# peter-seres/python-ray-tracer

Measured on AMD Instinct MI355X. Metric: Mrays/sec + frame time (ms) at 1920x1080, 8 spheres, depth=3, higher is better.
Workload: dtype f64

## Files before the change

python-ray-tracer_amd/csrc/rt_device.h:

```cpp
#pragma once
#include <hip/hip_runtime.h>
#include <stdint.h>
#include "rt_kparams.h"
#include "rt_math.h"
#include "rt_facing.h"
#include "rt_layout.h"

#pragma clang fp contract(off)

#ifndef RT_FAST_DIVSQRT
#define RT_FAST_DIVSQRT 1
#endif
#ifndef RT_FAST_NORMALIZE
#define RT_FAST_NORMALIZE 1
#endif
#ifndef RT_FACING_SKIP
#define RT_FACING_SKIP 1
#endif

namespace rt {

constexpr int TABLE_THREADS = 256;

__device__ __forceinline__ int div_by(int n, int d, unsigned M, unsigned sh)
// ... 662 lines not shown
    constexpr bool F32 = MODE >= 1;
    if (MODE >= 2 && lds.NC > 0 && (canchor < 0 || p.lanes_primary)) {
        if (canchor >= 0) lanes_closest<true>(lds, p, canchor, o, R, a, bestn, bidx);
        else lanes_closest<false>(lds, p, -1, o, R, a, bestn, bidx);
    } else
    for (int k0 = 0; k0 < S; k0 += 64) {
      const int n = (S - k0 < 64) ? S - k0 : 64;
      unsigned long long mask = cull_mask(lds, S, canchor, k0, n, o, R, p.extent2, -1);
      mask &= (n == 64) ? ~0ull : ((1ull << n) - 1ull);
      RT_MARK(1);
      while (mask) {
        const int k = k0 + __builtin_ctzll(mask);
        mask &= mask - 1ull;
        sphere_closest<F32>(lds, p, k, o, R, a, bestn, bidx);
      }
      RT_MARK(2);
    }
    double best = 999.0;
    int idx = -1, type = HIT_NONE;
    if (bidx >= 0) {
        const double t = div_inrange(bestn, a);
        if (best > t && t > 0.0) { best = t; idx = bidx; type = HIT_SPHERE; }
    }
    const double *pl = lds.recs() + (F32 ? 0 : opaque(p.S) * SPH_STRIDE);
    for (int k = 0; k < P; ++k) {
        const double *g = pl + k * PL_STRIDE;
        double den, num;
        plane_den_num(g, plane_code(p, k), o, d, den, num, lds.trim);
        if (!(__builtin_fabs(den) < 0.001)) {
            const double t = div_inrange(num, den);
            if (best > t && t > 0.0) { best = t; idx = k; type = HIT_PLANE; }
        }
    }
    t_out = best; idx_out = idx; type_out = type;
    RT_MARK(3);
}

__device__ __forceinline__ bool any_hit_masks(const Lds &lds, const KParams &p, const V3 &o, const V3 &d, int anchor, int self)
{
    const int P = opaque(p.P);
    const int S = p.S;
    const V3 R = renormalize_unit(d);
    const double a = dot3(R, R);
    RT_MARK(6);
    const int canchor = (opaque(p.anchors) > 0) ? anchor : -1;
    const lanemask live = lanes_where(true);
    const lanemask a_sane = lanes_where(a > 0.999999) & lanes_where(a < 1.000001);
    lanemask occ = 0ull;
    for (int k0 = 0; k0 < S; k0 += 64) {
      if (k0 > 0 && (live & ~occ) == 0ull) break;
      const int n = (S - k0 < 64) ? S - k0 : 64;
      unsigned long long mask = cull_mask(lds, S, canchor, k0, n, o, R, p.extent2, self);
      mask &= (n == 64) ? ~0ull : ((1ull << n) - 1ull);
      RT_MARK(7);
      while (mask) {
        const int k = k0 + __builtin_ctzll(mask);
        mask &= mask - 1ull;
        occ |= sphere_any_mask<false>(lds, k, o, R, a, a_sane);
        if (mask && (live & ~occ) == 0ull) break;
      }
      RT_MARK(8);
    }
    const double *pl = lds.recs() + opaque(p.S) * SPH_STRIDE;
    for (int k = 0; k < P; ++k) {
        if ((live & ~occ) == 0ull) break;
        const double *g = pl + k * PL_STRIDE;
        double den, num;
        plane_den_num(g, plane_code(p, k), o, d, den, num, true);
        const double an = __builtin_fabs(num), ad = __builtin_fabs(den);
        int sx = (int)(__builtin_bit_cast(unsigned long long, num) >> 32) ^ (int)(__builtin_bit_cast(unsigned long long, den) >> 32);
        asm("" : "+v"(sx));
        const lanemask ahead = lanes_where(!(ad < 0.001)) & lanes_where(sx >= 0) & lanes_where(an > 0.0);
        const lanemask sure = lanes_where(an < 998.0 * ad);
        occ |= ahead & sure;
        const lanemask edge = ahead & ~sure & ~occ;
        if (edge != 0ull) {
            bool h = false;
            if (lane_of(edge) && !(an > 1000.0 * ad)) { const double t = num / den; h = 999.0 > t && t > 0.0; }
            occ |= lanes_where(h);
        }
    }
    RT_MARK(9);
    return lane_of(occ);
}

template <int MODE>
// ... 5 lines not shown
    const V3 R = renormalize_unit(d);
    const double a = dot3(R, R);
    RT_MARK(6);
    const bool a_sane = (a > 0.999999 && a < 1.000001);
    bool occ = false;
    const int canchor = (opaque(p.anchors) > 0) ? anchor : -1;
    if (MODE >= 2 && lds.NC > 0 && lanes) {
        occ = (canchor >= 0) ? lanes_any<true>(lds, p, canchor, o, R, a, self) : lanes_any<false>(lds, p, -1, o, R, a, self);
    } else
    for (int k0 = 0; k0 < S; k0 += 64) {
      if (k0 > 0 && __builtin_amdgcn_ballot_w64(!occ) == 0ull) break;
      const int n = (S - k0 < 64) ? S - k0 : 64;
      unsigned long long mask = cull_mask(lds, S, canchor, k0, n, o, R, p.extent2, self);
      mask &= (n == 64) ? ~0ull : ((1ull << n) - 1ull);
      RT_MARK(7);
      while (mask) {
        const int k = k0 + __builtin_ctzll(mask);
        mask &= mask - 1ull;
        if (!occ) occ = sphere_any<(MODE >= 1)>(lds, k, o, R, a, a_sane);
        if (mask && __builtin_amdgcn_ballot_w64(!occ) == 0ull) break;
      }
      RT_MARK(8);
    }
    const double *pl = lds.recs() + (MODE >= 1 ? 0 : opaque(p.S) * SPH_STRIDE);
    for (int k = 0; k < P; ++k) {
        if (!occ) {
            const double *g = pl + k * PL_STRIDE;
            double den, num;
            plane_den_num(g, plane_code(p, k), o, d, den, num);
            if (!(__builtin_fabs(den) < 0.001)) {
                const double an = __builtin_fabs(num), ad = __builtin_fabs(den);
                const bool same_sign = (num > 0.0 && den > 0.0) || (num < 0.0 && den < 0.0);
                if (same_sign) {
                    if (an < 998.0 * ad) occ = true;
                    else if (!(an > 1000.0 * ad)) { const double t = num / den; if (999.0 > t && t > 0.0) occ = true; }
                }
            }
        }
    }
    RT_MARK(9);
    return occ;
}

template <bool COUNT> struct RayCount {
    __device__ __forceinline__ void closest(bool) {}
    __device__ __forceinline__ void hit(bool) {}
    __device__ __forceinline__ void shadow(bool, bool) {}
// ... 128 lines not shown
    double t = a > 1.0 ? one : a;
    const int nsharp = (int)((sky_i64 *)k)[12];
    if (nsharp > 0) {
        double q = 1.0 - t;
#pragma unroll 1
        for (int i = 0; i < nsharp; ++i) q = q * q;
        t = 1.0 - q;
    }
    const double zx = k[6], zy = k[7], zz = k[8], nx = k[9], ny = k[10], nz = k[11];
    V3 g{k[3] + t * (below ? nx : zx), k[4] + t * (below ? ny : zy), k[5] + t * (below ? nz : zz)};
    const double s = dot3(d, V3{k[13], k[14], k[15]});
    if (s > 0.0) {
        double q = s;
        const int nhalo = (int)((sky_i64 *)k)[23];
#pragma unroll 1
        for (int i = 0; i < nhalo; ++i) q = q * q;
        g = V3{g.x + k[20] * q, g.y + k[21] * q, g.z + k[22] * q};
    }
    if (s >= k[16]) g = V3{g.x + k[17], g.y + k[18], g.z + k[19]};
    return g;
}

__device__ __forceinline__ int hit_slot(int type, int idx, int S) { return (type == HIT_SPHERE) ? idx : S + idx; }
template <bool NOREC> __device__ __forceinline__ int plane_base(int S) { return NOREC ? 0 : S * SPH_STRIDE; }
template <bool NOREC>
__device__ __forceinline__ void hit_normal(const Lds &lds, int type, int idx, int plb, const V3 &Pt, V3 &N, V3 &bN)
{
    if (type == HIT_SPHERE) {
        const SphHot g = sphere_hot<NOREC>(lds, idx);
        N = normalize3(V3{Pt.x - g.x, Pt.y - g.y, Pt.z - g.z});
        bN = V3{0.0002 * N.x, 0.0002 * N.y, 0.0002 * N.z};
    } else {
        const double *g = lds.recs() + plb + idx * PL_STRIDE;
        N = V3{g[6], g[7], g[8]};
        bN = V3{g[9], g[10], g[11]};
    }
}

template <bool PARK, int WGT, bool COUNT, int MODE, class MS>
__device__ __forceinline__ void trace_bounce(const Lds &lds, const KParams &p, bool &alive, int anchor,
                                             V3 &o, V3 &d, V3 &rgb, RayCount<COUNT> &cnt, MS &ms, int b = 0)
{
    constexpr bool NOREC = MODE >= 1;
    constexpr bool FACING_SKIP = RT_FACING_SKIP != 0 && MODE != 2;
    const int S = p.S, P = p.P, L = opaque(p.L);
    rgb = V3{0.0, 0.0, 0.0};
    double t = 999.0; int idx = -1, type = HIT_NONE;
    cnt.closest(alive);
    RT_MARK(11);
    if (alive) closest_hit<MODE>(lds, p, o, d, MS::lens ? -1 : anchor, t, idx, type);
    if constexpr (MS::sky) {
        if (alive && type == HIT_NONE) rgb = sky_color(p.scene + (size_t)p.lens.sky, d);
    }
    alive = alive && (type != HIT_NONE);
    cnt.hit(alive);
    if (alive) {
        V3 Pt{o.x + t * d.x, o.y + t * d.y, o.z + t * d.z};
        const int plb = plane_base<NOREC>(NOREC ? 0 : opaque(S));
        const int coff = (type == HIT_SPHERE) ? idx * SPH_STRIDE + 4 : plb + idx * PL_STRIDE + 12;
        volatile const lds_f64 *colp = (volatile const lds_f64 *)lds.recs() + coff;
        volatile const double *colf = (NOREC && type == HIT_SPHERE) ? p.scene + coff : lds.recs() + coff;
        typedef __attribute__((address_space(3))) float lds_f32;
        volatile const lds_f32 *col1 = nullptr;
        if constexpr (MODE == 1) col1 = (volatile const lds_f32 *)lds.col32 + 4 * ((type == HIT_SPHERE) ? idx : (int)padS(S, lds.NC) + idx);
        unsigned texi = 0u;
        if constexpr (MS::tex) texi = texel_of(p, hit_slot(type, idx, S), Pt);
        auto texel = [&](int c) -> double { return (double)((volatile const float *)p.lens.texels)[4 * (size_t)texi + c]; };
        V3 colr{0.0, 0.0, 0.0};
        if constexpr (!PARK && MS::tex) {
            const f4 tc = reinterpret_cast<const f4 *>(p.lens.texels)[texi];
            colr = V3{(double)tc[0], (double)tc[1], (double)tc[2]};
        }
        else if constexpr (!PARK) colr = (MODE == 1) ? V3{(double)col1[0], (double)col1[1], (double)col1[2]} : V3{colf[0], colf[1], colf[2]};
        auto col = [&](int c) -> double {
            if constexpr (PARK && MS::tex) return texel(c);
            else if constexpr (PARK && MODE == 1) return (double)col1[c];
            else if constexpr (PARK && NOREC) return colf[c];
            else if constexpr (PARK) return colp[c];
            else return c == 0 ? colr.x : (c == 1 ? colr.y : colr.z);
        };
        auto lambert_add = [&](double k, const V3 &e) {
// ... 131 lines not shown
                if (!occluded) lambert_add(k, V3{1.0, 1.0, 1.0});
            }
        }
        d = dpark.get();
        if constexpr (MS::scat) {
            alive = refract_continue<WGT>(lds, ms, N, Pt, o, d, b < p.depth ? b : -1);
        } else if constexpr (MS::refr) {
            refract_continue<WGT>(lds, ms, N, Pt, o, d);
        } else {
        const V3 Rd = mirror_dir(d, N);
        o = V3{Pt.x + 0.0002 * Rd.x, Pt.y + 0.0002 * Rd.y, Pt.z + 0.0002 * Rd.z};
        d = Rd;
        }
        RT_MARK(10);
    }
}


template <bool PARK, int WGT, bool COUNT, int MODE, class MS>
__device__ __forceinline__ V3 sample(const Lds &lds, const KParams &p, bool alive, V3 o, V3 d, RayCount<COUNT> &cnt, MS &ms,
                                     unsigned key = 0u, unsigned lkey = 0u)
{
    Park3<PARK, WGT, MODE == 3> acc(lds.acc, 0, lds.wave);
    acc.set(V3{0.0, 0.0, 0.0});
    if constexpr (MS::mat) SLOT(W) = 1.0;
    if constexpr (MS::scat) SLOT(KEY) = (double)key;
    if constexpr (MS::soft) SLOT(LKEY) = (double)lkey;
    for (int b = 0; b <= p.depth; ++b) {
        if (__builtin_amdgcn_ballot_w64(alive) == 0ull) break;
        if constexpr (COUNT) {
            const unsigned long long am = __builtin_amdgcn_ballot_w64(alive);
            if ((threadIdx.x & 63u) == 0u && p.ray_counts) {
                atomicAdd(&p.ray_counts[4 + 2 * b], 1ull);
                atomicAdd(&p.ray_counts[5 + 2 * b], (unsigned long long)__builtin_popcountll(am));
            }
        }
        V3 rgb;
#ifdef RT_REGION_STATS
        ((volatile unsigned *)lds.reg)[(threadIdx.x >> 6) * 32 + 30] = b >= 2 ? 12u : 0u;
#endif
        trace_bounce<PARK, WGT, COUNT, MODE, MS>(lds, p, alive, b == 0 ? 0 : -1, o, d, rgb, cnt, ms, b);
        if (b == 0) acc.set(rgb);
        else {
            double wgt;
            if constexpr (MS::mat) wgt = SLOT(W); else wgt = p.refl_pow[b - 1];
            const V3 a = acc.get();
            acc.set(V3{a.x + wgt * rgb.x, a.y + wgt * rgb.y, a.z + wgt * rgb.z});
// ... 4 lines not shown
                *w = *w * SLOT(REFL);
            }
        }
    }
    return acc.get();
}

__device__ __forceinline__ V3 pixel_P(const KParams &p, int x, int y)
{
    if (p.pixel_loc) {
        const size_t wh = (size_t)p.w * p.h, o = (size_t)x * p.h + y;
        return V3{p.pixel_loc[o], p.pixel_loc[wh + o], p.pixel_loc[2 * wh + o]};
    }
    return V3{p.px, (double)x * p.dy + p.y0, (double)y * p.dz + p.z0};
}

__device__ __forceinline__ V3 lattice_P(const KParams &p, int i, int j)
{
    const double ya = (double)(i >> 1) * p.dy + p.y0, yb = (double)((i + 1) >> 1) * p.dy + p.y0;
    const double za = (double)(j >> 1) * p.dz + p.z0, zb = (double)((j + 1) >> 1) * p.dz + p.z0;
    return V3{p.px, (i & 1) ? 0.5 * ya + 0.5 * yb : ya, (j & 1) ? 0.5 * za + 0.5 * zb : za};
}

__device__ __forceinline__ V3 primary_dir(const KParams &p, const V3 &P)
{
    const V3 v{p.cam_R[0] * P.x + p.cam_R[1] * P.y + p.cam_R[2] * P.z,
               p.cam_R[3] * P.x + p.cam_R[4] * P.y + p.cam_R[5] * P.z,
               p.cam_R[6] * P.x + p.cam_R[7] * P.y + p.cam_R[8] * P.z};
    return normalize3(v);
}

__device__ __forceinline__ void lens_ray(const KParams &p, unsigned x, unsigned y, unsigned s, const V3 &P, V3 &o, V3 &d)
{
    const V3 v{p.cam_R[0] * P.x + p.cam_R[1] * P.y + p.cam_R[2] * P.z,
               p.cam_R[3] * P.x + p.cam_R[4] * P.y + p.cam_R[5] * P.z,
               p.cam_R[6] * P.x + p.cam_R[7] * P.y + p.cam_R[8] * P.z};
    const double t = p.lens.focus / P.x;
    const V3 F{p.cam_o[0] + t * v.x, p.cam_o[1] + t * v.y, p.cam_o[2] + t * v.z};
    const unsigned key = lens_key(x, y, s, p.seed);
    double u0 = 0.0, u1 = 0.0;
#pragma unroll 1
    for (int j = 0; j < 8; ++j) {
        const unsigned tj = (unsigned)j << 1;
        const double c0 = hash_unit(key, tj);
        const double c1 = hash_unit(key, tj | 1u);
        if (c0 * c0 + c1 * c1 < 1.0) { u0 = c0; u1 = c1; break; }
    }
    const double a0 = p.lens.aperture * u0, a1 = p.lens.aperture * u1;
    o = V3{(p.cam_o[0] + a0 * p.cam_R[1]) + a1 * p.cam_R[2], (p.cam_o[1] + a0 * p.cam_R[4]) + a1 * p.cam_R[5],
           (p.cam_o[2] + a0 * p.cam_R[7]) + a1 * p.cam_R[8]};
    d = normalize3(V3{F.x - o.x, F.y - o.y, F.z - o.z});
}

__device__ __forceinline__ void store_pixel(const KParams &p, long long off, long long fo, double R, double G, double B)
{
    if (p.out_u8) {
        const uint8_t r8 = clip_color(R), g8 = clip_color(G), b8 = clip_color(B);
        const uint8_t c1 = p.u8_rgb ? g8 : b8, c2 = p.u8_rgb ? b8 : g8;
        uint8_t *o8 = p.out_u8 + fo;
        if (p.u8_hwc) {
            const long long xr = off / p.h, yy = off - xr * p.h;
            uint8_t *px = o8 + (yy * p.plane_stride + xr) * 3;
            px[0] = r8; px[1] = c1; px[2] = c2;
        } else {
            o8[off] = r8;
            o8[p.plane_stride + off] = c1;
            o8[2 * p.plane_stride + off] = c2;
        }
    }
    if (p.out_f32) {
        float *o32 = p.out_f32 + fo;
        o32[off] = (float)R;
        o32[p.plane_stride + off] = (float)G;
        o32[2 * p.plane_stride + off] = (float)B;
    }
}

__global__ __launch_bounds__(TABLE_THREADS) void tables_kernel(const KParams p, float *__restrict__ out)
{
    const int nrec = (int)lds_doubles(p.S, p.P, p.L);
    const int Sp = padS(p.S, p.NC), NCp = pad4(p.NC);
    const TableLayout tl = table_layout(p.S, p.NC, p.anchors, p.P);
    float *sph32 = out;
    float *tab = out + tl.tab;
    float *csph32 = out + tl.csph32;
    float *ctab = out + tl.ctab;
    const double *rec = p.scene;
    const float NINF = -__builtin_inff();
    for (int k = threadIdx.x; k < Sp; k += TABLE_THREADS) {
        const double *g = rec + k * SPH_STRIDE;
        const bool real = k < p.S;
        sph32[4 * k + 0] = real ? (float)g[0] : 0.0f; sph32[4 * k + 1] = real ? (float)g[1] : 0.0f;
        sph32[4 * k + 2] = real ? (float)g[2] : 0.0f; sph32[4 * k + 3] = real ? (float)g[3] : NINF;
    }
    float *col32 = out + tl.col32;
    for (int k = threadIdx.x; k < Sp + pad4(p.P); k += TABLE_THREADS) {
        const double *g = k < p.S ? rec + k * SPH_STRIDE + 4 : rec + p.S * SPH_STRIDE + (k - Sp) * PL_STRIDE + 12;
// ... 81 lines not shown

template <Family F, int WSLOT, bool FRESH>
__device__ __forceinline__ MatState<F, WSLOT, FRESH> mat_state(double *matl, int M, int nsh = 1)
{
    typedef __attribute__((address_space(3))) double lds_d;
    typedef MatState<F, WSLOT, FRESH> MS;
    if constexpr (MS::mat) return MS{(unsigned)(size_t)(lds_d *)(matl + 1), (unsigned)(size_t)(lds_d *)(matl + 1 + MS::COLS * M), nsh};
    else return {};
}

__device__ __forceinline__ void tile_xy(const KParams &p, int tile, int &tx, int &ty)
{
    tx = div_by(tile, p.tiles_y, p.tiles_y_magic, p.tiles_y_shift);
    ty = tile - tx * p.tiles_y;
}

template <bool AA, bool PARK, int WPW, bool COUNT = false, bool LAT = false, int MODE = 0, Family F = Family::PLAIN>
__global__ __launch_bounds__(64 * WPW, MODE >= 2 ? RT_W_LANES : (AA ? (PARK ? RT_W_AAPARK : 4) : (PARK ? RT_W_PARK : 5))) void render_kernel(const KParams p)
{
    constexpr int WG_THREADS = 64 * WPW, WAVES_PER_WG = WPW;
    constexpr bool M2 = MODE >= 2;
    constexpr bool NOREC = MODE >= 1;
    constexpr bool MAT = has_mat(F), SCAT = has_scat(F), SOFT = has_soft(F), LENS = has_lens(F), TEX = has_tex(F);
    const int nrec = (int)lds_doubles(NOREC ? 0 : p.S, p.P, p.L);
    const double *rec_src = p.scene + (NOREC ? (size_t)p.S * SPH_STRIDE : 0);
    double *accum = lds_raw + nrec;
    int *offw = reinterpret_cast<int *>(accum + lds_slots(AA, PARK, M2, F) * WG_THREADS);
    float *sph32 = reinterpret_cast<float *>(offw + lds_offset_words(PARK, WG_THREADS));
    const TableLayout tl = table_layout(p.S, p.NC, p.anchors, p.P);
    const bool LANES = MODE >= 2 && p.anchors > 0;
    float *tab = sph32 + tl.tab;
    float *csph32 = LANES ? nullptr : sph32 + tl.csph32;
    float *ctab = sph32 + tl.ctab;
    float *cbox = sph32 + tl.cbox;
    const size_t ntab = MODE == 1 ? tl.total_col : (LANES ? tl.total_lanes : tl.total);
    unsigned *wgstat = reinterpret_cast<unsigned *>(sph32 + ntab);
    if (threadIdx.x == 0) { wgstat[0] = 0u; wgstat[1] = 0u; }
    {
        for (int i = threadIdx.x; i < nrec; i += WG_THREADS) lds_raw[i] = rec_src[i];
        const int nf4 = (int)(ntab / 4);
        const f4 *src = reinterpret_cast<const f4 *>(p.ftab);
        f4 *dst = reinterpret_cast<f4 *>(sph32);
        for (int i = threadIdx.x; i < nf4; i += WG_THREADS) dst[i] = src[i];
    }
#ifdef RT_REGION_STATS
    double *matl = reinterpret_cast<double *>(wgstat + 4 + WPW * 32);
#else
    double *matl = reinterpret_cast<double *>(wgstat + 4);
#endif
    int nmat = 0, nsh = 1;
    if constexpr (MAT) {
        const double *msrc = p.scene + ((LENS || TEX) ? (size_t)p.lens.mat : mat_offset(p.S, p.P, p.L, p.NC));
        nmat = (int)msrc[0];
        const int nm = (int)mat_doubles(nmat, p.S, p.P, F);
        for (int i = threadIdx.x; i < nm; i += WG_THREADS) matl[i] = msrc[i];
        if constexpr (SOFT) nsh = (int)msrc[nm - 1];
    }
    __syncthreads();
#ifdef RT_REGION_STATS
    const Lds lds{sph32, tab, csph32, ctab, cbox, sph32 + tl.gbox, sph32 + tl.gtab, MODE == 1 ? sph32 + tl.col32 : nullptr, WPW == 2 ? 0 : p.NC, __builtin_amdgcn_readfirstlane((int)(threadIdx.x >> 6)), MODE < 2, MODE >= 2, WPW == 2 && !MAT, wgstat + 4, accum};
    for (int i = threadIdx.x & 63; i < 32; i += 64) lds.reg[(threadIdx.x >> 6) * 32 + i] = 0u;
    if ((threadIdx.x & 63) == 0) lds.reg[(threadIdx.x >> 6) * 32 + 31] = (unsigned)__builtin_amdgcn_s_memtime();
#else
    const Lds lds{sph32, tab, csph32, ctab, cbox, sph32 + tl.gbox, sph32 + tl.gtab, MODE == 1 ? sph32 + tl.col32 : nullptr, WPW == 2 ? 0 : p.NC, __builtin_amdgcn_readfirstlane((int)(threadIdx.x >> 6)), MODE < 2, MODE >= 2, WPW == 2 && !MAT, accum};
#endif

    const int wave = threadIdx.x >> 6, lane = threadIdx.x & 63;
    int bid = (int)blockIdx.x;
    const unsigned *ord = p.order;
    if (p.nframes > 1) {
        const int frame = div_by(bid, p.bpf, p.bpf_magic, p.bpf_shift);
        bid -= frame * p.bpf;
        if (ord && frame < p.nframes - 1) ord += p.seq_offset;
    }
    const bool by_tile = WPW >= TILE_ORDER_MIN_WPW && p.order_tiles;
    const int block = by_tile ? bid : (ord ? (int)ord[bid] : bid);
    const int wave_u = __builtin_amdgcn_readfirstlane(wave);
    const int tile_v = by_tile ? (ord ? (int)ord[bid * WAVES_PER_WG + wave_u] : bid * WAVES_PER_WG + wave_u) : block * WAVES_PER_WG + wave;
    const int tile = WPW >= TILE_ORDER_MIN_WPW ? __builtin_amdgcn_readfirstlane(tile_v) : tile_v;
    if (tile >= p.ntiles) return;
    const unsigned long long t_begin = (p.tile_cycles || p.cost) ? __builtin_amdgcn_s_memtime() : 0ull;
    int tx, ty;
    tile_xy(p, tile, tx, ty);
    const int x = p.x0 + tx * TILE + (lane >> 3);
    const int y = ty * TILE + (lane & 7);
    bool inb = (x < p.x1) && (y < p.h);
    if constexpr (LAT) inb = inb && ((((x | y) & 1) == 0) || (x >= 1 && x <= p.w - 2 && y >= 1 && y <= p.h - 2));
    const int xc = inb ? x : p.x0, yc = inb ? y : 0;
    typedef __attribute__((address_space(3))) int lds_i32;
    constexpr bool OFF_REMAT = PARK && MODE == 3;
    volatile lds_i32 *offp = OFF_REMAT ? nullptr : (volatile lds_i32 *)offw + threadIdx.x;
    if constexpr (PARK && !OFF_REMAT) *offp = inb ? (x - p.x0) * p.h + y : -1;

    const V3 o{p.cam_o[0], p.cam_o[1], p.cam_o[2]};
    RayCount<COUNT> cnt;
    constexpr int WSLOT = lds_slots(AA, PARK, M2, Family::PLAIN);
    auto ms = mat_state<F, WSLOT, !PARK || MODE == 3>(matl, nmat, nsh);
    const unsigned sseed = SCAT ? p.seed : 0u;
    double R, G, B;
    if constexpr (!AA) {
        unsigned key = 0u, lkey = 0u;
        if constexpr (SCAT) key = LAT ? scatter_key((unsigned)xc, (unsigned)yc, 0u, sseed) : scatter_key(2u * xc, 2u * yc, 0u, sseed);
        if constexpr (SOFT) lkey = LAT ? soft_key((unsigned)xc, (unsigned)yc, 0u, sseed) : soft_key(2u * xc, 2u * yc, 0u, sseed);
        const V3 P0 = LAT ? lattice_P(p, xc, yc) : pixel_P(p, xc, yc);
        V3 ro = o, rd;
        if constexpr (LENS) lens_ray(p, LAT ? (unsigned)xc : 2u * xc, LAT ? (unsigned)yc : 2u * yc, 0u, P0, ro, rd);
        else rd = primary_dir(p, P0);
        const V3 c = sample<PARK, WG_THREADS, COUNT, MODE, decltype(ms)>(lds, p, inb, ro, rd, cnt, ms, key, lkey);
        R = c.x; G = c.y; B = c.z;
    } else {
        const bool stoch = (p.aa == 2);
        const bool interior = !stoch && inb && x >= 1 && x <= p.w - 2 && y >= 1 && y <= p.h - 2;
        const int ntaps = stoch ? p.spp : ((__builtin_amdgcn_ballot_w64(interior) != 0ull) ? 9 : 1);
        constexpr unsigned NBX = 0x8858u, NBY = 0x0A25u;
        Park3<PARK && !M2, WG_THREADS> taps(lds.acc, 2);
#pragma unroll 1
        for (int tap = 0; tap < ntaps; ++tap) {
            const V3 Pp = pixel_P(p, xc, yc);
            V3 Pt = Pp;
            unsigned key = 0u, lkey = 0u;
            unsigned lx = 2u * xc, ly = 2u * yc;
            if constexpr (SCAT) key = scatter_key(2u * xc, 2u * yc, stoch ? (unsigned)tap : 0u, sseed);
            if constexpr (SOFT) lkey = soft_key(2u * xc, 2u * yc, stoch ? (unsigned)tap : 0u, sseed);
            if (stoch) {
                const unsigned hh = jitter_hash((unsigned)xc, (unsigned)yc, (unsigned)tap, p.seed);
                const double u = (double)(hh & 0xFFFFu) * 0x1p-16 + (0x1p-17 - 0.5);
                const double v = (double)(hh >> 16) * 0x1p-16 + (0x1p-17 - 0.5);
                Pt = V3{Pp.x, Pp.y + u * p.dy, Pp.z + v * p.dz};
            } else if (tap) {
                const int k = tap - 1;
// ... 11 lines not shown
            if (tap == 0) taps.set(s);
            else if (stoch) { const V3 a = taps.get(); taps.set(V3{a.x + s.x, a.y + s.y, a.z + s.z}); }
            else if (interior) { const V3 a = taps.get(); taps.set(V3{a.x + s.x, a.y + s.z, a.z + s.y}); }
        }
        { const V3 a = taps.get(); R = a.x; G = a.y; B = a.z; }
        if (stoch) { const double n = (double)p.spp; R = R / n; G = G / n; B = B / n; }
        else if (interior) { R = R / 9; G = G / 9; B = B / 9; }
    }

    long long off;
    if constexpr (OFF_REMAT) {
        const int l2 = (int)fresh_lane();
        const int x2 = p.x0 + tx * TILE + (l2 >> 3), y2 = ty * TILE + (l2 & 7);
        bool inb2 = (x2 < p.x1) && (y2 < p.h);
        if constexpr (LAT) inb2 = inb2 && ((((x2 | y2) & 1) == 0) || (x2 >= 1 && x2 <= p.w - 2 && y2 >= 1 && y2 <= p.h - 2));
        off = inb2 ? (long long)((x2 - p.x0) * p.h + y2) : -1ll;
    } else if constexpr (PARK) off = *offp; else off = inb ? (long long)(x - p.x0) * p.h + y : -1ll;
    if (off >= 0) {
        if constexpr (LAT) {
            double *q = p.out_f64 + off * 3;
            q[0] = R; q[1] = G; q[2] = B;
        } else {
            const long long fo = opaque(p.nframes) > 1 ? (long long)div_by((int)blockIdx.x, p.bpf, p.bpf_magic, p.bpf_shift) * p.frame_stride : 0ll;
            store_pixel(p, off, fo, R, G, B);
        }
    }
#ifdef RT_REGION_STATS
    RT_MARK(11);
    if (p.tile_cycles && (threadIdx.x & 63) < 24)
        atomicAdd(p.tile_cycles + p.ntiles + 16 + (threadIdx.x & 63), lds.reg[(threadIdx.x >> 6) * 32 + (threadIdx.x & 63)] >> 6);
#endif
    if constexpr (COUNT) {
        unsigned v[4] = {cnt.n_closest, cnt.n_issued, cnt.n_skipped, cnt.n_hit};
#pragma unroll
        for (int c = 0; c < 4; ++c) {
#pragma unroll
            for (int d = 32; d >= 1; d >>= 1) v[c] += __shfl_down(v[c], d);
            if ((threadIdx.x & 63) == 0 && p.ray_counts) atomicAdd(&p.ray_counts[c], (unsigned long long)v[c]);
        }
    }
    if ((p.tile_cycles || p.cost) && (threadIdx.x & 63) == 0) {
        const unsigned cyc = (unsigned)(__builtin_amdgcn_s_memtime() - t_begin);
        if (p.tile_cycles) p.tile_cycles[tile] = cyc;
        if (p.cost) {
            if (by_tile) p.cost[tile] = cyc >> 2;
            else {
                const int expected = (p.ntiles - block * WAVES_PER_WG < WAVES_PER_WG) ? p.ntiles - block * WAVES_PER_WG : WAVES_PER_WG;
// ... 1 lines not shown
                if ((int)atomicAdd(&wgstat[1], 1u) == expected - 1) p.cost[block] = atomicAdd(&wgstat[0], 0u);
            }
        }
    }
}

__global__ __launch_bounds__(256) void aa_resolve_kernel(const KParams p)
{
    const long long idx = (long long)blockIdx.x * 256 + threadIdx.x;
    if (idx >= (long long)(p.x1 - p.x0) * p.h) return;
    const int xr = (int)(idx / p.h), y = (int)(idx - (long long)xr * p.h), x = p.x0 + xr;
    const double *c = p.out_f64 + ((size_t)(2 * x - p.lat_x0) * p.lat_h + 2 * y) * 3;
    double R = c[0], G = c[1], B = c[2];
    if (x >= 1 && x <= p.w - 2 && y >= 1 && y <= p.h - 2) {
        constexpr unsigned NBX = 0x8858u, NBY = 0x0A25u;
#pragma unroll
        for (int k = 0; k < 8; ++k) {
            const int ddx = (int)((NBX >> (2 * k)) & 3u) - 1, ddy = (int)((NBY >> (2 * k)) & 3u) - 1;
            const double *s = c + ((long long)ddx * p.lat_h + ddy) * 3;
            R += s[0]; G += s[2]; B += s[1];
        }
        R = R / 9; G = G / 9; B = B / 9;
    }
    store_pixel(p, idx, 0ll, R, G, B);
}

__global__ __launch_bounds__(ORDER_THREADS) void order_kernel(const unsigned *__restrict__ cost, unsigned *__restrict__ gtmp,
                                                               unsigned *__restrict__ btmp, unsigned *__restrict__ order, int nblocks, int gshift,
                                                               int wshift, int nvalid)
{
    const unsigned wm = (1u << wshift) - 1u;
    auto place = [&](unsigned x, unsigned t, unsigned tail_) -> unsigned {
        return x < (unsigned)ORDER_XCDS ? ((((unsigned)ORDER_XCDS * (t >> wshift) + x) << wshift) | (t & wm)) : tail_ + t;
    };
    auto cost_of = [&](int it) -> unsigned { return it < nvalid ? cost[it] : 0u; };
    __shared__ unsigned hist[(ORDER_XCDS + 1) * ORDER_BUCKETS];
    __shared__ unsigned scan[ORDER_THREADS / 64];
    static_assert(ORDER_THREADS == ORDER_BUCKETS, "thread i owns bucket 1023 - i");
    const int i = threadIdx.x, lane = i & 63, wv = i >> 6;
    const int gb = 1 << gshift;
    const int full = nblocks >> gshift;
    const int rows = full / ORDER_XCDS;
    auto scan_classes = [&](int nc) {
        for (int c = 0; c < nc; ++c) {
            __syncthreads();
            const unsigned v = hist[c * ORDER_BUCKETS + ORDER_BUCKETS - 1 - i];
            unsigned incl = v;
// ... 84 lines not shown
```

python-ray-tracer_amd/csrc/rt_kparams.h:

```cpp
#pragma once
#include <stdint.h>

namespace rt {

struct KParams {
    const double *scene;
    const double *pixel_loc;
    uint8_t *out_u8;
    float *out_f32;
    unsigned *tile_cycles;
    unsigned *cost;
    const unsigned *order;
    int order_tiles;
    int seq_offset;
    int nframes, bpf;
    long long frame_stride;
    const float *ftab;
    unsigned long long *ray_counts;
    double *out_f64;
    int lattice;
    int lat_x0, lat_h;
    long long plane_stride;
    int w, h, x0, x1;
    int S, P, L, depth;
    int NC;
    unsigned plane_codes;
// ... 1 lines not shown
    unsigned tiles_y_magic, tiles_y_shift, bpf_magic, bpf_shift;
    int anchors, spp;
    unsigned seed;
    int u8_hwc;
    int lanes_primary;
    float extent2, floor_anch;
    double px, y0, dy, z0, dz;
    double cam_o[3];
    double cam_R[9];
    double amb, lamb;
    double facing_tau;
    union {
        double refl_pow[16];
        struct {
            double aperture;
            double focus;
            long long mat;
            long long tex;
            const float *texels;
            long long lit;
            long long sky;
        } lens;
    };
};

}
```

python-ray-tracer_amd/csrc/rt_launch.h:

```cpp
#pragma once
#include "rt_kparams.h"
#include "rt_facing.h"
#include "rt_plan.h"

#include <cmath>
#include <cstring>

#ifdef __clang__
#pragma clang fp contract(off)
#endif

namespace rt {

struct View {
    double cam_o[3] = {0, 0, 0}, cam_R[9] = {0};
    int w = 0, h = 0;
    double px = 0, y0 = 0, dy = 0, z0 = 0, dz = 0;
    double lens_a = 0.0, lens_f = 1.0;
    bool have_cam = false, have_grid = false, explicit_grid = false;
};

inline double reach_of(KParams &k, const double cam_o[3], double aperture, int depth, double extent2)
{
    double cam2 = cam_o[0] * cam_o[0] + cam_o[1] * cam_o[1] + cam_o[2] * cam_o[2];
    if (aperture > 0.0) { const double e = std::sqrt(cam2) + aperture; cam2 = e * e; }
    k.extent2 = (float)(1.0001 * (cam2 > extent2 ? cam2 : extent2));
    const double reach = std::sqrt(cam2) + 999.0 * (depth + 1) + std::sqrt(extent2);
    k.floor_anch = (float)(0x1p-39 * reach * reach);
    return reach;
}

inline double frame_part(KParams &k, const View &v, const SceneLayout &lay, const double *scene, const double *pixel_loc, int lanes_primary,
                         int x0, int x1, double aperture, int depth)
{
    std::memset(&k, 0, sizeof k);
    k.scene = scene;
    k.nframes = 1;
    k.pixel_loc = v.explicit_grid ? pixel_loc : nullptr;
    k.w = v.w; k.h = v.h; k.x0 = x0; k.x1 = x1;
    k.S = lay.S; k.P = lay.P; k.L = lay.L; k.NC = lay.NC; k.plane_codes = lay.plane_codes;
    k.lanes_primary = lanes_primary;
    k.tiles_y = (int)rt_geo_tiles(v.h);
    k.px = v.px; k.y0 = v.y0; k.dy = v.dy; k.z0 = v.z0; k.dz = v.dz;
    std::memcpy(k.cam_o, v.cam_o, sizeof k.cam_o);
    std::memcpy(k.cam_R, v.cam_R, sizeof k.cam_R);
    k.anchors = anchors_of(lay);
    return reach_of(k, v.cam_o, aperture, depth, lay.extent2);
}

inline void guides_part(KParams &k, const View &v, const SceneLayout &lay, const double *scene, const double *pixel_loc, const float *texels,
                        int lanes_primary, int x0, int x1, void *d_guides, long long plane_stride)
{
    frame_part(k, v, lay, scene, pixel_loc, lanes_primary, x0, x1, 0.0, 0);
    k.out_f32 = (float *)d_guides;
    k.plane_stride = plane_stride;
    if (lay.T > 0) { k.lens.tex = lay.tex_off; k.lens.texels = texels; }
}

inline void render_part(KParams &k, const View &v, const SceneLayout &lay, Family fam, const rt_params *p, const double *scene,
                        const double *pixel_loc, const float *texels, int lanes_primary, int x0, int x1, void *d_u8, void *d_f32,
                        long long plane_stride, unsigned *tile_cycles)
{
    const bool lens = has_lens(fam);
    const double reach = frame_part(k, v, lay, scene, pixel_loc, lanes_primary, x0, x1, lens ? v.lens_a : 0.0, p->depth);
    k.out_u8 = (uint8_t *)d_u8;
    k.out_f32 = (float *)d_f32;
    k.tile_cycles = tile_cycles;
    k.plane_stride = plane_stride;
    k.depth = p->depth;
// ... 115 lines not shown
```

python-ray-tracer_amd/csrc/rt_layout.h:

```cpp
#pragma once
#include <stddef.h>

#ifdef __HIPCC__
#define RT_HD __host__ __device__
#else
#define RT_HD
#endif

#ifndef RT_W_PARK
#define RT_W_PARK 7
#endif
#ifndef RT_W_AAPARK
#define RT_W_AAPARK 7
#endif
#ifndef RT_W_LANES
#define RT_W_LANES 4
#endif

namespace rt {

constexpr int TILE = 8;
constexpr int TILE_ORDER_MIN_WPW = 4;
constexpr int BOX_STRIDE = 8;
constexpr int CULL_STRIDE = 4;
// ... 11 lines not shown
#endif
constexpr int CLUSTER_MIN = RT_CLUSTER_MIN;
constexpr int SUPER = 8;
constexpr int TEX_STRIDE = 20;
constexpr int SKY_DOUBLES = 24;

enum class Family { PLAIN, MAT, REFR, SCAT, SOFT, LENS, LENS_SOFT, TEX_SCAT, TEX_SOFT, TEX_LENS, TEX_LENS_SOFT,
                    LIT_SCAT, LIT_SOFT, LIT_LENS, LIT_LENS_SOFT, SKY_SCAT, SKY_SOFT, SKY_LENS, SKY_LENS_SOFT };
constexpr int FAMILIES = 19;
RT_HD constexpr bool has_mat(Family f) { return f != Family::PLAIN; }
RT_HD constexpr bool has_refr(Family f) { return f >= Family::REFR; }
RT_HD constexpr bool has_scat(Family f) { return f >= Family::SCAT; }
RT_HD constexpr bool has_soft(Family f) { return f == Family::SOFT || f == Family::LENS_SOFT || f == Family::TEX_SOFT || f == Family::TEX_LENS_SOFT || f == Family::LIT_SOFT || f == Family::LIT_LENS_SOFT || f == Family::SKY_SOFT || f == Family::SKY_LENS_SOFT; }
RT_HD constexpr bool has_lens(Family f) { return f == Family::LENS || f == Family::LENS_SOFT || f == Family::TEX_LENS || f == Family::TEX_LENS_SOFT || f == Family::LIT_LENS || f == Family::LIT_LENS_SOFT || f == Family::SKY_LENS || f == Family::SKY_LENS_SOFT; }
RT_HD constexpr bool has_tex(Family f) { return f >= Family::TEX_SCAT; }
RT_HD constexpr bool has_lit(Family f) { return f >= Family::LIT_SCAT; }
RT_HD constexpr bool has_sky(Family f) { return f >= Family::SKY_SCAT; }
RT_HD constexpr int table_cols(Family f) { return has_scat(f) ? 6 : (has_refr(f) ? 5 : 3); }

RT_HD inline int pad4(int n) { return (n + 3) & ~3; }
RT_HD inline int supers(int NC) { return (NC + SUPER - 1) / SUPER; }

RT_HD inline size_t lds_doubles(int S, int P, int L) { return (size_t)S * SPH_STRIDE + (size_t)P * PL_STRIDE + (size_t)L * LT_STRIDE; }
RT_HD inline size_t mat_offset(int S, int P, int L, int NC) { return lds_doubles(S, P, L) + (size_t)(NC + supers(NC)) * CL_STRIDE + 1; }
RT_HD inline size_t mat_doubles(int M, int S, int P, Family f) { return M > 0 ? 1 + (size_t)table_cols(f) * M + ((size_t)S + P + 1) / 2 + (has_soft(f) ? 1 : 0) : 0; }
RT_HD inline size_t tex_doubles(int T) { return T > 0 ? 1 + (size_t)TEX_STRIDE * T : 0; }
RT_HD inline size_t lit_doubles(int S, int P, int L) { return (size_t)LT_STRIDE * L + 2 * ((size_t)S + P); }

RT_HD inline int padS(int S, int NC) { return NC > 0 ? NC * CLUSTER : pad4(S); }

RT_HD constexpr int lds_slots(bool aa, bool park, bool mode2, Family f) { return (park ? ((aa && !mode2) ? 9 : 6) : 0) + (has_mat(f) ? 3 : 0) + (has_refr(f) ? 4 : 0) + (has_scat(f) ? 2 : 0) + (has_soft(f) ? 1 : 0); }
RT_HD inline int lds_offset_words(bool park, int wgt) { return park ? wgt : 0; }
struct TableLayout { size_t tab, ctab, cbox, gbox, gtab, csph32, total_lanes, total, col32, total_col; };
RT_HD inline TableLayout table_layout(int S, int NC, int anchors, int P = 0)
{
    const size_t Sp = padS(S, NC), NCp = pad4(NC), NG = supers(NC), NGp = pad4((int)NG);
    TableLayout t;
    size_t o = 4 * Sp;
    t.tab = o;    o += (size_t)anchors * Sp * CULL_STRIDE;
    t.ctab = o;   o += (size_t)anchors * NCp * CULL_STRIDE;
    t.cbox = o;   o += NCp * BOX_STRIDE;
    t.gbox = o;   o += NG * BOX_STRIDE;
    t.gtab = o;   o += (size_t)anchors * NGp * CULL_STRIDE;
    t.total_lanes = o;
    t.csph32 = o; o += 4 * NCp;
    t.total = o;
// ... 32 lines not shown
```

python-ray-tracer_amd/csrc/rt_math.h:

```cpp
#pragma once
#include <stdint.h>

#ifdef __HIPCC__
#define RT_MATH_FN __host__ __device__ __forceinline__
#else
#define RT_MATH_FN static inline
#endif

#ifdef __clang__
#pragma clang fp contract(off)
#endif

namespace rt {

struct V3 { double x, y, z; };
struct F3 { float x, y, z; };

RT_MATH_FN double dot3(const V3 &a, const V3 &b) { return a.x * b.x + a.y * b.y + a.z * b.z; }

RT_MATH_FN V3 normalize3_generic(const V3 &v)
{
    double n = __builtin_sqrt(v.x * v.x + v.y * v.y + v.z * v.z);
    return V3{v.x / n, v.y / n, v.z / n};
}
// ... 58 lines not shown
    h = (h ^ x) * 0x85EBCA6Bu; h ^= h >> 13;
    h = (h ^ y) * 0xC2B2AE35u; h ^= h >> 16;
    return h;
}
RT_MATH_FN unsigned scatter_hash(unsigned key, unsigned t)
{
    unsigned h = (key ^ t) * 0x27D4EB2Fu; h ^= h >> 15;
    h *= 0x165667B1u; h ^= h >> 13;
    return h;
}

RT_MATH_FN unsigned jitter_hash(unsigned x, unsigned y, unsigned s, unsigned seed) { return scatter_hash(hash_xy(seed, x, y), s); }

RT_MATH_FN unsigned scatter_key(unsigned x, unsigned y, unsigned s, unsigned seed) { return hash_xy(seed ^ 0x5CA77E12u, x, y) ^ (s << 9); }

RT_MATH_FN unsigned soft_key(unsigned x, unsigned y, unsigned s, unsigned seed) { return hash_xy(seed ^ 0x50F7117Eu, x, y) ^ (s << 20); }

RT_MATH_FN unsigned lens_key(unsigned x, unsigned y, unsigned s, unsigned seed) { return hash_xy(seed ^ 0x1E45D0F5u, x, y) ^ (s << 4); }

RT_MATH_FN double hash_unit(unsigned key, unsigned t) { return (double)(scatter_hash(key, t) >> 8) * 0x1p-23 + (0x1p-24 - 1.0); }

RT_MATH_FN uint8_t clip_color(double c)
{
    if (!(c == c)) return 0;
    if (c <= -0.5) return 0;
    if (c >= 255.5) return 255;
    const int i = (int)__builtin_rint(c);
    return (uint8_t)(i < 0 ? 0 : (i > 255 ? 255 : i));
}

}
```

Before: 214,800.

## Precompute fixed layout offsets and camera grid on host; trim kernel prologue

Adds a KFixed block to the kernel parameters with host-precomputed LDS record counts, plane base offset, table layout offsets and a pre-scaled camera matrix, so the kernel no longer recomputes table_layout and offsets per workgroup in non-M2 modes. It also builds primary directions incrementally from grid coordinates, single-pass loads the LDS prologue when the tables fit in one workgroup, skips accumulator init and wgstat zeroing when unused, makes the tile index always wave-uniform, and simplifies pixel storing and color clipping with a branchless fmin/fmax. These cut scalar and prologue overhead at the cost of a larger kernel argument block. Color clipping now maps NaN through fmin/fmax instead of an explicit check, and rint rounding differs slightly at the edges.

Result: no change. 216,500 (median of 6 runs) (+0.8%).

```diff
diff --git a/python-ray-tracer_amd/csrc/rt_device.h b/python-ray-tracer_amd/csrc/rt_device.h
--- a/python-ray-tracer_amd/csrc/rt_device.h
+++ b/python-ray-tracer_amd/csrc/rt_device.h
@@ -708,7 +708,7 @@
         const double t = div_inrange(bestn, a);
         if (best > t && t > 0.0) { best = t; idx = bidx; type = HIT_SPHERE; }
     }
-    const double *pl = lds.recs() + (F32 ? 0 : opaque(p.S) * SPH_STRIDE);
+    const double *pl = lds.recs() + (F32 ? 0 : opaque(p.fx.plb));
     for (int k = 0; k < P; ++k) {
         const double *g = pl + k * PL_STRIDE;
         double den, num;
@@ -747,7 +747,7 @@
       }
       RT_MARK(8);
     }
-    const double *pl = lds.recs() + opaque(p.S) * SPH_STRIDE;
+    const double *pl = lds.recs() + opaque(p.fx.plb);
     for (int k = 0; k < P; ++k) {
         if ((live & ~occ) == 0ull) break;
         const double *g = pl + k * PL_STRIDE;
@@ -799,7 +799,7 @@
       }
       RT_MARK(8);
     }
-    const double *pl = lds.recs() + (MODE >= 1 ? 0 : opaque(p.S) * SPH_STRIDE);
+    const double *pl = lds.recs() + (MODE >= 1 ? 0 : opaque(p.fx.plb));
     for (int k = 0; k < P; ++k) {
         if (!occ) {
             const double *g = pl + k * PL_STRIDE;
@@ -974,7 +974,6 @@
 }
 
 __device__ __forceinline__ int hit_slot(int type, int idx, int S) { return (type == HIT_SPHERE) ? idx : S + idx; }
-template <bool NOREC> __device__ __forceinline__ int plane_base(int S) { return NOREC ? 0 : S * SPH_STRIDE; }
 template <bool NOREC>
 __device__ __forceinline__ void hit_normal(const Lds &lds, int type, int idx, int plb, const V3 &Pt, V3 &N, V3 &bN)
 {
@@ -1008,7 +1007,7 @@
     cnt.hit(alive);
     if (alive) {
         V3 Pt{o.x + t * d.x, o.y + t * d.y, o.z + t * d.z};
-        const int plb = plane_base<NOREC>(NOREC ? 0 : opaque(S));
+        const int plb = NOREC ? 0 : opaque(p.fx.plb);
         const int coff = (type == HIT_SPHERE) ? idx * SPH_STRIDE + 4 : plb + idx * PL_STRIDE + 12;
         volatile const lds_f64 *colp = (volatile const lds_f64 *)lds.recs() + coff;
         volatile const double *colf = (NOREC && type == HIT_SPHERE) ? p.scene + coff : lds.recs() + coff;
@@ -1186,7 +1185,7 @@
                                      unsigned key = 0u, unsigned lkey = 0u)
 {
     Park3<PARK, WGT, MODE == 3> acc(lds.acc, 0, lds.wave);
-    acc.set(V3{0.0, 0.0, 0.0});
+    if constexpr (MODE >= 2) acc.set(V3{0.0, 0.0, 0.0});
     if constexpr (MS::mat) SLOT(W) = 1.0;
     if constexpr (MS::scat) SLOT(KEY) = (double)key;
     if constexpr (MS::soft) SLOT(LKEY) = (double)lkey;
@@ -1237,12 +1236,28 @@
     return V3{p.px, (i & 1) ? 0.5 * ya + 0.5 * yb : ya, (j & 1) ? 0.5 * za + 0.5 * zb : za};
 }
 
+__device__ __forceinline__ V3 cam_times(const KParams &p, const V3 &P)
+{
+    return V3{p.cam_R[0] * P.x + p.cam_R[1] * P.y + p.cam_R[2] * P.z,
+              p.cam_R[3] * P.x + p.cam_R[4] * P.y + p.cam_R[5] * P.z,
+              p.cam_R[6] * P.x + p.cam_R[7] * P.y + p.cam_R[8] * P.z};
+}
 __device__ __forceinline__ V3 primary_dir(const KParams &p, const V3 &P)
 {
-    const V3 v{p.cam_R[0] * P.x + p.cam_R[1] * P.y + p.cam_R[2] * P.z,
-               p.cam_R[3] * P.x + p.cam_R[4] * P.y + p.cam_R[5] * P.z,
-               p.cam_R[6] * P.x + p.cam_R[7] * P.y + p.cam_R[8] * P.z};
-    return normalize3(v);
+    return normalize3(cam_times(p, P));
+}
+
+__device__ __forceinline__ V3 cam_rows_xy(const KParams &p, const V3 &P)
+{
+    return V3{p.cam_R[0] * P.x + p.cam_R[1] * P.y, p.cam_R[3] * P.x + p.cam_R[4] * P.y, p.cam_R[6] * P.x + p.cam_R[7] * P.y};
+}
+__device__ __forceinline__ V3 cam_rows_xy_grid(const KParams &p, double Py)
+{
+    return V3{p.fx.cam_Rg[0] + p.fx.cam_Rg[3] * Py, p.fx.cam_Rg[1] + p.fx.cam_Rg[4] * Py, p.fx.cam_Rg[2] + p.fx.cam_Rg[5] * Py};
+}
+__device__ __forceinline__ V3 cam_rows_z(const KParams &p, const V3 &a, double Pz)
+{
+    return V3{a.x + p.fx.cam_Rg[6] * Pz, a.y + p.fx.cam_Rg[7] * Pz, a.z + p.fx.cam_Rg[8] * Pz};
 }
 
 __device__ __forceinline__ void lens_ray(const KParams &p, unsigned x, unsigned y, unsigned s, const V3 &P, V3 &o, V3 &d)
@@ -1267,27 +1282,41 @@
     d = normalize3(V3{F.x - o.x, F.y - o.y, F.z - o.z});
 }
 
+template <bool SELECTS>
 __device__ __forceinline__ void store_pixel(const KParams &p, long long off, long long fo, double R, double G, double B)
 {
+    const long long ps = p.plane_stride;
     if (p.out_u8) {
         const uint8_t r8 = clip_color(R), g8 = clip_color(G), b8 = clip_color(B);
-        const uint8_t c1 = p.u8_rgb ? g8 : b8, c2 = p.u8_rgb ? b8 : g8;
         uint8_t *o8 = p.out_u8 + fo;
-        if (p.u8_hwc) {
+        const bool rgb = p.u8_rgb != 0;
+        if constexpr (SELECTS) {
+            const uint8_t c1 = rgb ? g8 : b8, c2 = rgb ? b8 : g8;
+            if (p.u8_hwc) {
+                const long long xr = off / p.h, yy = off - xr * p.h;
+                uint8_t *px = o8 + (yy * ps + xr) * 3;
+                px[0] = r8; px[1] = c1; px[2] = c2;
+            } else {
+                o8[off] = r8;
+                o8[ps + off] = c1;
+                o8[2 * ps + off] = c2;
+            }
+        } else if (p.u8_hwc) {
             const long long xr = off / p.h, yy = off - xr * p.h;
-            uint8_t *px = o8 + (yy * p.plane_stride + xr) * 3;
-            px[0] = r8; px[1] = c1; px[2] = c2;
+            uint8_t *px = o8 + (yy * ps + xr) * 3;
+            px[0] = r8; px[rgb ? 1 : 2] = g8; px[rgb ? 2 : 1] = b8;
         } else {
+            uint8_t *og = o8 + (rgb ? ps : 2 * ps), *ob = o8 + (rgb ? 2 * ps : ps);
             o8[off] = r8;
-            o8[p.plane_stride + off] = c1;
-            o8[2 * p.plane_stride + off] = c2;
+            og[off] = g8;
+            ob[off] = b8;
         }
     }
     if (p.out_f32) {
-        float *o32 = p.out_f32 + fo;
+        float *o32 = p.out_f32 + fo, *o32g = o32 + ps, *o32b = o32 + 2 * ps;
         o32[off] = (float)R;
-        o32[p.plane_stride + off] = (float)G;
-        o32[2 * p.plane_stride + off] = (float)B;
+        o32g[off] = (float)G;
+        o32b[off] = (float)B;
     }
 }
 
@@ -1415,26 +1444,45 @@
     constexpr bool M2 = MODE >= 2;
     constexpr bool NOREC = MODE >= 1;
     constexpr bool MAT = has_mat(F), SCAT = has_scat(F), SOFT = has_soft(F), LENS = has_lens(F), TEX = has_tex(F);
-    const int nrec = (int)lds_doubles(NOREC ? 0 : p.S, p.P, p.L);
-    const double *rec_src = p.scene + (NOREC ? (size_t)p.S * SPH_STRIDE : 0);
+    const KFixed &fx = p.fx;
+    const int nrec = M2 ? (int)lds_doubles(0, p.P, p.L) : (NOREC ? fx.nrec_norec : fx.nrec);
+    const double *rec_src = p.scene + (NOREC ? (M2 ? (size_t)p.S * SPH_STRIDE : (size_t)fx.plb) : 0);
     double *accum = lds_raw + nrec;
     int *offw = reinterpret_cast<int *>(accum + lds_slots(AA, PARK, M2, F) * WG_THREADS);
     float *sph32 = reinterpret_cast<float *>(offw + lds_offset_words(PARK, WG_THREADS));
-    const TableLayout tl = table_layout(p.S, p.NC, p.anchors, p.P);
+    const TableLayout tlk = table_layout(p.S, p.NC, p.anchors, p.P);
+    struct { size_t tab, ctab, cbox, gbox, gtab, csph32, col32; } tl{(size_t)fx.tab, (size_t)fx.ctab, (size_t)fx.cbox, (size_t)fx.gbox, (size_t)fx.gtab, (size_t)fx.csph32, (size_t)fx.col32};
+    if constexpr (M2) { tl.tab = tlk.tab; tl.ctab = tlk.ctab; tl.cbox = tlk.cbox; tl.gbox = tlk.gbox; tl.gtab = tlk.gtab; tl.csph32 = tlk.csph32; tl.col32 = tlk.col32; }
     const bool LANES = MODE >= 2 && p.anchors > 0;
     float *tab = sph32 + tl.tab;
     float *csph32 = LANES ? nullptr : sph32 + tl.csph32;
     float *ctab = sph32 + tl.ctab;
     float *cbox = sph32 + tl.cbox;
-    const size_t ntab = MODE == 1 ? tl.total_col : (LANES ? tl.total_lanes : tl.total);
-    unsigned *wgstat = reinterpret_cast<unsigned *>(sph32 + ntab);
-    if (threadIdx.x == 0) { wgstat[0] = 0u; wgstat[1] = 0u; }
+    const int nf4 = M2 ? (int)((LANES ? tlk.total_lanes : tlk.total) / 4) : (MODE == 1 ? fx.nf4_col : fx.nf4);
+    unsigned *wgstat = reinterpret_cast<unsigned *>(sph32 + (M2 ? (LANES ? tlk.total_lanes : tlk.total) : (size_t)4 * nf4));
+    constexpr bool SMALL = WPW == 2;
+    if constexpr (SMALL) {
+        if (p.cost) {
+            asm volatile("");
+            if (threadIdx.x == 0) { wgstat[0] = 0u; wgstat[1] = 0u; }
+        }
+    } else if (threadIdx.x == 0) { wgstat[0] = 0u; wgstat[1] = 0u; }
     {
-        for (int i = threadIdx.x; i < nrec; i += WG_THREADS) lds_raw[i] = rec_src[i];
-        const int nf4 = (int)(ntab / 4);
         const f4 *src = reinterpret_cast<const f4 *>(p.ftab);
         f4 *dst = reinterpret_cast<f4 *>(sph32);
-        for (int i = threadIdx.x; i < nf4; i += WG_THREADS) dst[i] = src[i];
+        if (SMALL && nrec <= WG_THREADS && nf4 <= WG_THREADS) {
+            const int i = threadIdx.x;
+            const bool hr = i < nrec, hf = i < nf4;
+            double r;
+            f4 t;
+            if (hr) r = rec_src[i];
+            if (hf) t = src[i];
+            if (hr) lds_raw[i] = r;
+            if (hf) dst[i] = t;
+        } else {
+            for (int i = threadIdx.x; i < nrec; i += WG_THREADS) lds_raw[i] = rec_src[i];
+            for (int i = threadIdx.x; i < nf4; i += WG_THREADS) dst[i] = src[i];
+        }
     }
 #ifdef RT_REGION_STATS
     double *matl = reinterpret_cast<double *>(wgstat + 4 + WPW * 32);
@@ -1470,7 +1518,7 @@
     const int block = by_tile ? bid : (ord ? (int)ord[bid] : bid);
     const int wave_u = __builtin_amdgcn_readfirstlane(wave);
     const int tile_v = by_tile ? (ord ? (int)ord[bid * WAVES_PER_WG + wave_u] : bid * WAVES_PER_WG + wave_u) : block * WAVES_PER_WG + wave;
-    const int tile = WPW >= TILE_ORDER_MIN_WPW ? __builtin_amdgcn_readfirstlane(tile_v) : tile_v;
+    const int tile = __builtin_amdgcn_readfirstlane(tile_v);
     if (tile >= p.ntiles) return;
     const unsigned long long t_begin = (p.tile_cycles || p.cost) ? __builtin_amdgcn_s_memtime() : 0ull;
     int tx, ty;
@@ -1495,10 +1543,19 @@
         unsigned key = 0u, lkey = 0u;
         if constexpr (SCAT) key = LAT ? scatter_key((unsigned)xc, (unsigned)yc, 0u, sseed) : scatter_key(2u * xc, 2u * yc, 0u, sseed);
         if constexpr (SOFT) lkey = LAT ? soft_key((unsigned)xc, (unsigned)yc, 0u, sseed) : soft_key(2u * xc, 2u * yc, 0u, sseed);
-        const V3 P0 = LAT ? lattice_P(p, xc, yc) : pixel_P(p, xc, yc);
         V3 ro = o, rd;
-        if constexpr (LENS) lens_ray(p, LAT ? (unsigned)xc : 2u * xc, LAT ? (unsigned)yc : 2u * yc, 0u, P0, ro, rd);
-        else rd = primary_dir(p, P0);
+        if constexpr (LENS) {
+            const V3 P0 = LAT ? lattice_P(p, xc, yc) : pixel_P(p, xc, yc);
+            lens_ray(p, LAT ? (unsigned)xc : 2u * xc, LAT ? (unsigned)yc : 2u * yc, 0u, P0, ro, rd);
+        } else if constexpr (M2) rd = primary_dir(p, LAT ? lattice_P(p, xc, yc) : pixel_P(p, xc, yc));
+        else {
+            V3 a;
+            double Pz;
+            if constexpr (LAT) { const V3 P0 = lattice_P(p, xc, yc); a = cam_rows_xy_grid(p, P0.y); Pz = P0.z; }
+            else if (p.pixel_loc) { const V3 P0 = pixel_P(p, xc, yc); a = cam_rows_xy(p, P0); Pz = P0.z; }
+            else { a = cam_rows_xy_grid(p, (double)xc * p.dy + p.y0); Pz = (double)yc * p.dz + p.z0; }
+            rd = normalize3(cam_rows_z(p, a, Pz));
+        }
         const V3 c = sample<PARK, WG_THREADS, COUNT, MODE, decltype(ms)>(lds, p, inb, ro, rd, cnt, ms, key, lkey);
         R = c.x; G = c.y; B = c.z;
     } else {
@@ -1556,7 +1613,7 @@
             q[0] = R; q[1] = G; q[2] = B;
         } else {
             const long long fo = opaque(p.nframes) > 1 ? (long long)div_by((int)blockIdx.x, p.bpf, p.bpf_magic, p.bpf_shift) * p.frame_stride : 0ll;
-            store_pixel(p, off, fo, R, G, B);
+            store_pixel<M2>(p, off, fo, R, G, B);
         }
     }
 #ifdef RT_REGION_STATS
@@ -1604,7 +1661,7 @@
         }
         R = R / 9; G = G / 9; B = B / 9;
     }
-    store_pixel(p, idx, 0ll, R, G, B);
+    store_pixel<false>(p, idx, 0ll, R, G, B);
 }
 
 __global__ __launch_bounds__(ORDER_THREADS) void order_kernel(const unsigned *__restrict__ cost, unsigned *__restrict__ gtmp,
diff --git a/python-ray-tracer_amd/csrc/rt_kparams.h b/python-ray-tracer_amd/csrc/rt_kparams.h
--- a/python-ray-tracer_amd/csrc/rt_kparams.h
+++ b/python-ray-tracer_amd/csrc/rt_kparams.h
@@ -2,6 +2,16 @@
 #include <stdint.h>
 
 namespace rt {
+
+struct KFixed {
+    int nrec, nrec_norec;
+    int plb;
+    int ltb, ltb_norec;
+    int nf4, nf4_lanes, nf4_col;
+    int tab, ctab, cbox, gbox, gtab, csph32, col32;
+    int pad_;
+    double cam_Rg[9];
+};
 
 struct KParams {
     const double *scene;
@@ -49,6 +59,7 @@
             long long sky;
         } lens;
     };
+    KFixed fx;
 };
 
 }
diff --git a/python-ray-tracer_amd/csrc/rt_launch.h b/python-ray-tracer_amd/csrc/rt_launch.h
--- a/python-ray-tracer_amd/csrc/rt_launch.h
+++ b/python-ray-tracer_amd/csrc/rt_launch.h
@@ -30,6 +30,20 @@
     return reach;
 }
 
+inline void fixed_part(KFixed &f, int S, int P, int L, int NC, int anchors, const double cam_R[9], double px)
+{
+    const TableLayout t = table_layout(S, NC, anchors, P);
+    f.nrec = (int)lds_doubles(S, P, L); f.nrec_norec = (int)lds_doubles(0, P, L);
+    f.plb = S * SPH_STRIDE;
+    f.ltb = f.plb + P * PL_STRIDE; f.ltb_norec = P * PL_STRIDE;
+    f.nf4 = (int)(t.total / 4); f.nf4_lanes = (int)(t.total_lanes / 4); f.nf4_col = (int)(t.total_col / 4);
+    f.tab = (int)t.tab; f.ctab = (int)t.ctab; f.cbox = (int)t.cbox; f.gbox = (int)t.gbox; f.gtab = (int)t.gtab;
+    f.csph32 = (int)t.csph32; f.col32 = (int)t.col32;
+    f.pad_ = 0;
+    for (int c = 0; c < 3; ++c)
+        for (int r = 0; r < 3; ++r) f.cam_Rg[3 * c + r] = c == 0 ? cam_R[3 * r] * px : cam_R[3 * r + c];
+}
+
 inline double frame_part(KParams &k, const View &v, const SceneLayout &lay, const double *scene, const double *pixel_loc, int lanes_primary,
                          int x0, int x1, double aperture, int depth)
 {
@@ -45,6 +59,7 @@
     std::memcpy(k.cam_o, v.cam_o, sizeof k.cam_o);
     std::memcpy(k.cam_R, v.cam_R, sizeof k.cam_R);
     k.anchors = anchors_of(lay);
+    fixed_part(k.fx, k.S, k.P, k.L, k.NC, k.anchors, k.cam_R, k.px);
     return reach_of(k, v.cam_o, aperture, depth, lay.extent2);
 }
 
diff --git a/python-ray-tracer_amd/csrc/rt_layout.h b/python-ray-tracer_amd/csrc/rt_layout.h
--- a/python-ray-tracer_amd/csrc/rt_layout.h
+++ b/python-ray-tracer_amd/csrc/rt_layout.h
@@ -57,6 +57,7 @@
 RT_HD inline int supers(int NC) { return (NC + SUPER - 1) / SUPER; }
 
 RT_HD inline size_t lds_doubles(int S, int P, int L) { return (size_t)S * SPH_STRIDE + (size_t)P * PL_STRIDE + (size_t)L * LT_STRIDE; }
+template <bool NOREC> RT_HD inline int plane_base(int S) { return NOREC ? 0 : S * SPH_STRIDE; }
 RT_HD inline size_t mat_offset(int S, int P, int L, int NC) { return lds_doubles(S, P, L) + (size_t)(NC + supers(NC)) * CL_STRIDE + 1; }
 RT_HD inline size_t mat_doubles(int M, int S, int P, Family f) { return M > 0 ? 1 + (size_t)table_cols(f) * M + ((size_t)S + P + 1) / 2 + (has_soft(f) ? 1 : 0) : 0; }
 RT_HD inline size_t tex_doubles(int T) { return T > 0 ? 1 + (size_t)TEX_STRIDE * T : 0; }
diff --git a/python-ray-tracer_amd/csrc/rt_math.h b/python-ray-tracer_amd/csrc/rt_math.h
--- a/python-ray-tracer_amd/csrc/rt_math.h
+++ b/python-ray-tracer_amd/csrc/rt_math.h
@@ -104,11 +104,7 @@
 
 RT_MATH_FN uint8_t clip_color(double c)
 {
-    if (!(c == c)) return 0;
-    if (c <= -0.5) return 0;
-    if (c >= 255.5) return 255;
-    const int i = (int)__builtin_rint(c);
-    return (uint8_t)(i < 0 ? 0 : (i > 255 ? 255 : i));
+    return (uint8_t)(int)__builtin_rint(__builtin_fmin(__builtin_fmax(c, 0.0), 255.0));
 }
 
 }
```
